# debbiemarkslab/BEAR

Measured on AMD Instinct MI355X. Metric: k-mer contexts/sec (DM-marginal+grad h), k=13, higher is better.
Workload: dtype f64

## Files before the change

bear_amd/csrc/kernels_plan.h:

```cpp
#pragma once
#include "plan_common.h"

__global__ __launch_bounds__(256) void plan_scan_kernel(const uint32_t *__restrict__ counts, uint64_t n_rows, int ncol,
                                                        uint8_t *__restrict__ quad_light,
                                                        unsigned long long *__restrict__ heavy_counts,
                                                        unsigned long long *__restrict__ hist) {
  __shared__ uint32_t s_heavy[3];
  __shared__ uint32_t s_hist[2 * SRT_NKEY];
  __shared__ uint32_t s_big[PLN_NBIG + 1];
  __shared__ unsigned long long s_total, s_cells;
  __shared__ uint32_t s_cmax;
  unsigned long long my_total = 0ull;
  uint32_t my_cells = 0u, my_cmax = 0u;
  if (threadIdx.x == 0) {
    s_total = s_cells = 0ull;
    s_cmax = 0u;
  }
  if (threadIdx.x < 3) s_heavy[threadIdx.x] = 0;
  if (threadIdx.x < 2 * SRT_NKEY) s_hist[threadIdx.x] = 0;
  for (uint32_t k = threadIdx.x; k <= PLN_NBIG; k += 256) s_big[k] = 0;
  __syncthreads();
  const uint64_t n_quads = (n_rows + PLN_QUAD - 1) / PLN_QUAD;
  for (uint64_t g = (uint64_t)blockIdx.x * 256 + threadIdx.x; g < n_quads; g += (uint64_t)gridDim.x * 256) {
    uint32_t light = 0, qhc = 0, qhr = 0;
// ... 156 lines not shown
    meta[2] = run > 0xffffffffull ? 1ull : 0ull;
  }
  __syncthreads();
  unsigned long long off = part[threadIdx.x];
  for (uint64_t t = lo; t < hi; ++t) {
    tiles[t].off16 = (uint32_t)off;
    off += tiles[t].blk16;
  }
}

__global__ __launch_bounds__(1024) void plan_fill_kernel(const uint32_t *__restrict__ counts, uint64_t n_rows, int ncol,
                                                         const pln_tile *__restrict__ tiles, uint64_t n_tiles,
                                                         unsigned char *__restrict__ stream,
                                                         pln_heavy_col *__restrict__ heavy_col,
                                                         pln_heavy_row *__restrict__ heavy_row,
                                                         uint64_t *__restrict__ heavy_stop,
                                                         unsigned long long *__restrict__ cursors) {
  constexpr int RPT = (PLN_RMAX + 1023) / 1024;
  __shared__ uint32_t hist[SRT_NHIST];
  __shared__ uint32_t offs[SRT_NHIST];
  __shared__ uint32_t scan[16];
  __shared__ uint16_t sorted[PLN_NI + 64];
  __shared__ uint32_t s_hc, s_hr;
#ifdef BEAR_DET_BUILD
  __shared__ uint32_t comp[PLN_NI];
  static_assert((PLN_NI & (PLN_NI - 1)) == 0 && PLN_NI <= 2048, "bitonic sort over the tile's items: PLN_NI / 2 pairs, at most one per thread");
  __shared__ unsigned long long hkey[PLN_HCAP], htmp[PLN_HCAP];
#endif
  const uint32_t tid = threadIdx.x, rep = tid & (SRT_REP - 1);
  for (uint64_t t = blockIdx.x; t < n_tiles; t += gridDim.x) {
    const pln_tile ti = tiles[t];
    const uint32_t rows = ti.rows_items >> 16, n_light = ti.rows_items & 0xffffu;
    const uint32_t hc_cap = ti.hc_hr >> 16, hr_cap = ti.hc_hr & 0xffffu;
    const pln_layout L = pln_block_layout(rows, n_light, hc_cap, hr_cap);
    unsigned char *blk = stream + (size_t)ti.off16 * 16;
    uint16_t *E = reinterpret_cast<uint16_t *>(blk);
    uint8_t *nrow = blk + L.nrow;
    uint16_t *items = reinterpret_cast<uint16_t *>(blk + L.items);
    uint16_t *hoff = reinterpret_cast<uint16_t *>(blk + L.hoff);
    uint32_t *hcnt = reinterpret_cast<uint32_t *>(blk + L.hcnt);
    uint16_t *hrow = reinterpret_cast<uint16_t *>(blk + L.hrow);
    double *hn = reinterpret_cast<double *>(blk + L.hn);
    if (tid < SRT_NHIST) hist[tid] = 0;
    if (tid == 0) {
      s_hc = 0;
      s_hr = 0;
    }
    __syncthreads();
#ifdef BEAR_DET_BUILD
    uint32_t det_hc[RPT], det_hr[RPT];
    {
      uint32_t base_c = 0, base_r = 0;
#pragma unroll
      for (int k = 0; k < RPT; ++k) {
        const uint32_t lr = tid + 1024u * k;
        uint32_t nc = 0, nr = 0;
        if (lr < rows) {
          double n = 0.0;
          for (int b = 0; b < 5; ++b) {
            const uint32_t cv = counts[(ti.row0 + lr) * 5 + b];
            n += (double)cv;
            nc += (b < ncol && cv > SRT_CL) ? 1u : 0u;
          }
          nr = n > (double)SRT_CL ? 1u : 0u;
        }
        const uint32_t packed = nc | (nr << 16);
        const int lane = tid & 63, wave = tid >> 6;
        uint32_t incl = packed;
#pragma unroll
        for (int off = 1; off < 64; off <<= 1) {
          const uint32_t o = (uint32_t)__shfl_up((int)incl, off, 64);
          if (lane >= off) incl += o;
        }
        __syncthreads();
        if (lane == 63) scan[wave] = incl;
        __syncthreads();
        uint32_t before = 0, total = 0;
        for (int w = 0; w < 16; ++w) {
          if (w < wave) before += scan[w];
          total += scan[w];
        }
        const uint32_t excl = before + incl - packed;
        det_hc[k] = base_c + (excl & 0xffffu);
        det_hr[k] = base_r + (excl >> 16);
        base_c += total & 0xffffu;
        base_r += total >> 16;
      }
      __syncthreads();
      if (tid == 0) {
        s_hc = base_c;
        s_hr = base_r;
      }
    }
#endif
    uint32_t c[RPT][5], rank[RPT][5];
#pragma unroll
    for (int k = 0; k < RPT; ++k) {
      const uint32_t lr = tid + 1024u * k;
#pragma unroll
      for (int b = 0; b < 5; ++b) {
        c[k][b] = 0;
        rank[k][b] = 0;
      }
      if (lr < rows) {
        const uint64_t r = ti.row0 + lr;
        double n = 0.0;
#pragma unroll
        for (int b = 0; b < 5; ++b) {
          c[k][b] = counts[r * 5 + b];
          n += (double)c[k][b];
        }
        nrow[lr] = n < 1.0 ? (uint8_t)0 : (n <= (double)SRT_CL ? (uint8_t)n : (uint8_t)255);
        if (n > (double)SRT_CL) {
#ifdef BEAR_DET_BUILD
          const uint32_t k2 = hr_cap ? det_hr[k] : 0xffffffffu;
#else
          const uint32_t k2 = hr_cap ? atomicAdd(&s_hr, 1u) : 0xffffffffu;
#endif
          if (k2 < hr_cap) {
            hrow[k2] = (uint16_t)lr;
            hn[k2] = n;
          } else {
            const unsigned long long q = atomicAdd(&cursors[1], 1ull);
            heavy_row[q].row = r;
            heavy_row[q].n = n;
          }
        }
        if (ncol == 4 && c[k][4] > SRT_CL) heavy_stop[atomicAdd(&cursors[2], 1ull)] = c[k][4];
#pragma unroll
        for (int b = 0; b < 5; ++b) {
          if (b >= ncol) c[k][b] = 0;
          if (c[k][b] > SRT_CL) {
#ifdef BEAR_DET_BUILD
            const uint32_t k2 = hc_cap ? det_hc[k]++ : 0xffffffffu;
#else
            const uint32_t k2 = hc_cap ? atomicAdd(&s_hc, 1u) : 0xffffffffu;
#endif
            if (k2 < hc_cap) {
              hoff[k2] = (uint16_t)(lr * 5 + b);
              hcnt[k2] = c[k][b];
            } else {
              const unsigned long long q = atomicAdd(&cursors[0], 1ull);
              heavy_col[q].off = r * 5 + b;
              heavy_col[q].c = c[k][b];
            }
            c[k][b] = 0;
          }
          if (c[k][b] != 0) rank[k][b] = atomicAdd(&hist[(c[k][b] - 1) * SRT_REP + rep], 1u);
        }
      } else if (lr < ((rows + 15u) & ~15u)) {
        nrow[lr] = 0;
      }
    }
    __syncthreads();
    {
      const uint32_t v = tid < SRT_NHIST ? hist[tid] : 0u;
      const int lane = tid & 63, wave = tid >> 6;
      uint32_t incl = v;
#pragma unroll
      for (int off = 1; off < 64; off <<= 1) {
        uint32_t o = (uint32_t)__shfl_up((int)incl, off, 64);
        if (lane >= off) incl += o;
      }
      if (lane == 63) scan[wave] = incl;
      __syncthreads();
      uint32_t base = 0;
      for (int w = 0; w < wave; ++w) base += scan[w];
      if (tid < SRT_NHIST) offs[tid] = base + incl - v;
    }
    __syncthreads();
    if (tid < 30) E[tid] = (uint16_t)(tid < SRT_CL ? offs[tid * SRT_REP] : n_light);
    if (tid == 30) E[30] = (uint16_t)hc_cap;
    if (tid == 31) E[31] = (uint16_t)hr_cap;
#pragma unroll
    for (int k = 0; k < RPT; ++k)
#pragma unroll
      for (int b = 0; b < 5; ++b)
        if (c[k][b] != 0) sorted[offs[(c[k][b] - 1) * SRT_REP + rep] + rank[k][b]] = (uint16_t)((tid + 1024u * k) * 5 + b);
    __syncthreads();
#ifdef BEAR_DET_BUILD
    {
      for (uint32_t i = tid; i < PLN_NI; i += 1024) {
        uint32_t key = 0;
        for (uint32_t q = 1; q < SRT_CL; ++q) key += offs[q * SRT_REP] <= i ? 1u : 0u;
        comp[i] = i < n_light ? (key << 16) | sorted[i] : 0xffffffffu;
      }
      __syncthreads();
      for (uint32_t size = 2; size <= PLN_NI; size <<= 1)
        for (uint32_t stride = size >> 1; stride > 0; stride >>= 1) {
          const uint32_t lo = 2u * tid - (tid & (stride - 1u)), hi = lo + stride;
          if (tid < PLN_NI / 2) {
            const bool up = (lo & size) == 0u;
            const uint32_t a = comp[lo], bq = comp[hi];
            if ((a > bq) == up) {
              comp[lo] = bq;
              comp[hi] = a;
            }
          }
          __syncthreads();
        }
      for (uint32_t i = tid; i < n_light; i += 1024) sorted[i] = (uint16_t)(comp[i] & 0xffffu);
      __syncthreads();
      const uint32_t nhc = s_hc < hc_cap ? s_hc : hc_cap, nhr = s_hr < hr_cap ? s_hr : hr_cap;
      if (tid < nhc) hkey[tid] = ((unsigned long long)hoff[tid] << 32) | hcnt[tid];
      __syncthreads();
      if (tid < nhc) {
        uint32_t r = 0;
        for (uint32_t q = 0; q < nhc; ++q) r += hkey[q] < hkey[tid] ? 1u : 0u;
        htmp[r] = hkey[tid];
      }
      __syncthreads();
      if (tid < nhc) {
        hoff[tid] = (uint16_t)(htmp[tid] >> 32);
        hcnt[tid] = (uint32_t)htmp[tid];
      }
      __syncthreads();
      if (tid < nhr) hkey[tid] = ((unsigned long long)hrow[tid] << 48) | tid;
      if (tid < nhr) htmp[tid] = (unsigned long long)__double_as_longlong(hn[tid]);
      __syncthreads();
      uint32_t r = 0;
      unsigned long long mine = 0ull, myn = 0ull;
      if (tid < nhr) {
        for (uint32_t q = 0; q < nhr; ++q) r += hkey[q] < hkey[tid] ? 1u : 0u;
        mine = hkey[tid];
        myn = htmp[tid];
      }
      __syncthreads();
      if (tid < nhr) {
        hrow[r] = (uint16_t)(mine >> 48);
        hn[r] = __longlong_as_double((long long)myn);
      }
      __syncthreads();
    }
#endif
    const uint32_t padded = (n_light + 63u) & ~63u;
    for (uint32_t i = tid; i < padded; i += 1024) items[i] = i < n_light ? sorted[i] : (uint16_t)PLN_SENTINEL;
    __syncthreads();
  }
}

__global__ __launch_bounds__(1024) void plan_live_kernel(const pln_tile *__restrict__ tiles, uint64_t n_tiles,
                                                         const unsigned char *__restrict__ stream, uint16_t *__restrict__ live) {
  constexpr int RPT = (PLN_RMAX + 1023) / 1024;
  __shared__ uint32_t cnt[RPT * 16];
  const uint32_t tid = threadIdx.x, lane = tid & 63, wave = tid >> 6;
  for (uint64_t t = blockIdx.x; t < n_tiles; t += gridDim.x) {
    const pln_tile ti = tiles[t];
    const uint32_t rows = ti.rows_items >> 16;
    const uint8_t *nrow = stream + (size_t)ti.off16 * 16 + 64;
    uint16_t *out = live + t * PLN_LIVE_STRIDE;
    unsigned long long mask[RPT];
#pragma unroll
    for (int k = 0; k < RPT; ++k) {
      const uint32_t lr = tid + 1024u * k;
      mask[k] = __builtin_amdgcn_ballot_w64(lr < rows && nrow[lr] != 0);
      if (lane == 0) cnt[k * 16 + wave] = (uint32_t)__builtin_popcountll(mask[k]);
    }
    __syncthreads();
    uint32_t total = 0;
#pragma unroll
    for (int k = 0; k < RPT; ++k) {
      uint32_t base = total;
      for (int w = 0; w < 16; ++w) {
        const uint32_t c = cnt[k * 16 + w];
        if (w < (int)wave) base += c;
        total += c;
      }
      if ((mask[k] >> lane) & 1ull) out[1 + base + (uint32_t)__builtin_popcountll(mask[k] & ((1ull << lane) - 1ull))] = (uint16_t)(tid + 1024u * k);
    }
    if (tid == 0) out[0] = (uint16_t)total;
    __syncthreads();
  }
}

template <bool NORM, bool AR>
__global__ __launch_bounds__(PLN_THREADS, 4) void dm_prior_plan_kernel(const double *__restrict__ prior,
                                                                                    uint64_t n_rows, bear_params prm_arg,
                                                                                    pln_view pv,
                                                                                    const double2 *__restrict__ logtab_g,
                                                                                    double *__restrict__ partials,
                                                                                    const bear_step_io io
#ifdef PLN_STAMPS
                                                                                    , unsigned long long *__restrict__ dbg
#endif
                                                                                    ) {
  extern __shared__ __attribute__((aligned(16))) unsigned char srt_smem[];
  pln_lds_n &S = *reinterpret_cast<pln_lds_n *>(srt_smem);
  const bear_params prm = bear_params_of(prm_arg, io);
  const uint32_t tid = threadIdx.x, lane = tid & 63, wave = srt_uniform(tid >> 6);
  const double u = prm.inv_h, eps = prm.eps, eps5 = 5.0 * prm.eps;
  double acc[2] = {0.0, 0.0};

  if (tid < BEAR_LOGTAB_N) S.logtab[tid] = logtab_g[tid];
  if (tid < SRT_NKEY) {
    const bear_dp o = srt_general_fast(u + eps5, (double)(tid + 1), logtab_g);
    S.tabD[tid] = o.D;
    S.tabP[tid] = o.P;
  }
  if (tid < PLN_NBUF) {
    S.buf[tid].pri[PLN_SENTINEL] = 1.0;
    S.ticket[tid] = PLN_TICKET_START(PLN_WAVES - PLN_DMA_WAVES);
    S.sum_fail[tid] = 0xffffffffu;
  }

  const bool dma_wave = wave >= PLN_WAVES - PLN_DMA_WAVES;
  const uint32_t dw = wave - (PLN_WAVES - PLN_DMA_WAVES);
  constexpr bool GEN = !NORM && !AR;
  constexpr bool NT = GEN && PLN_GEN_NT;
  auto stage = [&](const pln_tile &ti, uint32_t b, bool with_nrow) {
    const uint32_t rows = ti.rows_items >> 16;
    if (rows == 0) return;
    const uint32_t pbytes = (rows * 40u) & ~15u, bbytes = ti.blk16 * 16u;
    const unsigned char *psrc = reinterpret_cast<const unsigned char *>(prior + ti.row0 * 5);
    const unsigned char *bsrc = pv.stream + (size_t)ti.off16 * 16;
    if (GEN && dw == 0 && lane == 0) S.nrow_in[b] = with_nrow ? 1u : 0u;
    if (!GEN || with_nrow) {
      for (uint32_t pc = dw; (pc << 10) < bbytes; pc += PLN_DMA_WAVES) pln_dma_piece<NT>(S.buf[b].blk, bsrc, bbytes, pc, lane);
    } else {
      const uint32_t items0 = pln_block_layout(rows, ti.rows_items & 0xffffu, ti.hc_hr >> 16, ti.hc_hr & 0xffffu).items;
      if (dw == PLN_DMA_WAVES - 1) pln_dma_piece<NT>(S.buf[b].blk, bsrc, 64u, 0u, lane);
      for (uint32_t pc = dw; (pc << 10) < bbytes - items0; pc += PLN_DMA_WAVES)
        pln_dma_piece<NT>(S.buf[b].blk + items0, bsrc + items0, bbytes - items0, pc, lane);
    }
    for (uint32_t pc = dw; (pc << 10) < pbytes; pc += PLN_DMA_WAVES) pln_dma_piece<NT>(S.buf[b].pri, psrc, pbytes, pc, lane);
    if (dw == 0 && ((rows * 40u) & 15u)) {
      const __attribute__((address_space(4))) double *tail =
          (const __attribute__((address_space(4))) double *)(uintptr_t)(prior + (ti.row0 + rows) * 5 - 1);
      const double v = *tail;
      if (lane == 0) S.buf[b].pri[rows * 5 - 1] = v;
    }
  };

  constexpr uint32_t PF_INSTR = (NORM || AR || PLN_GEN_PREFETCH) ? PLN_PREFETCH_KIB / 8u : 0u;
  auto prefetch_behind = [&](const pln_tile &ti) -> uint32_t {
    const uint32_t rows = ti.rows_items >> 16;
    if (PF_INSTR == 0 || rows == 0) return 0u;
    const uint64_t end_bytes = n_rows * 40ull, base = (ti.row0 + rows) * 40ull;
    const uint32_t m = srt_uniform((uint32_t)(uintptr_t)S.pf_scratch);
    uint32_t issued = 0;
    for (uint32_t k = dw; k < PF_INSTR; k += PLN_DMA_WAVES) {
      uint64_t off = base + ((uint64_t)(k * 64u + lane) << 7);
      if (off + 4u > end_bytes) off = end_bytes - 4u;
      const unsigned char *g = reinterpret_cast<const unsigned char *>(prior) + off;
      uint32_t keep_m0;
      asm volatile("s_mov_b32 %0, m0\n\ts_mov_b32 m0, %2\n\ts_nop 0\n\tglobal_load_lds_dword %1, off\n\ts_mov_b32 m0, %0"
                   : "=&s"(keep_m0)
                   : "v"(g), "s"(m)
                   : "memory");
      ++issued;
    }
    return issued;
  };
  uint32_t pf_young = 0;
#ifdef PLN_STAMPS
  unsigned long long tph[8] = {0, 0, 0, 0, 0, 0, 0, 0}, t_prev = __builtin_amdgcn_s_memtime();
  int prev_kind = 0;
#define PLN_STAMP(k)                                              \
  {                                                               \
    const unsigned long long now = __builtin_amdgcn_s_memtime();  \
    tph[k] += now - t_prev;                                       \
    t_prev = now;                                                 \
  }
#else
#define PLN_STAMP(k)
#endif
  static_assert(PLN_NBUF == 2, "the DMA-wave protocol below is written for a two-slot ring");
  const uint64_t G = gridDim.x;
  const uint64_t first = (pv.n_tiles * (uint64_t)blockIdx.x) / G, count = (pv.n_tiles * ((uint64_t)blockIdx.x + 1)) / G - first;
  auto fetch_desc = [&](uint64_t j0) {
    if (dw == 0 && j0 < count)
      pln_dma_piece(S.desc[(j0 >> 5) & 1u], pv.tiles + first + j0, PLN_DESC_CHUNK * (uint32_t)sizeof(pln_tile), 0u, lane);
  };
  if (dma_wave) {
    __builtin_amdgcn_s_setprio(3);
    fetch_desc(0);
    fetch_desc(PLN_DESC_CHUNK);
    srt_wait_dma();
  }
  __syncthreads();
  pln_tile cur = pln_desc(S.desc, 0, count), nxt = pln_desc(S.desc, 1, count);
  if (dma_wave) stage(cur, 0, !PLN_GEN_NROW_ON_DEMAND);
  uint32_t slot = 0;
  for (uint64_t j = 0; j < count; ++j) {
#ifdef PLN_STAMPS
    PLN_STAMP(prev_kind)
    prev_kind = 4;
#endif
    if (dma_wave) pln_wait_all_but(pf_young);
    PLN_STAMP(1)
    srt_sync();
    PLN_STAMP(2)
    const pln_tile nn = pln_desc(S.desc, j + 2, count);
    if (dma_wave) {
      if ((j & (PLN_DESC_CHUNK - 1)) == 0 && j != 0) fetch_desc(j + PLN_DESC_CHUNK);
      stage(nxt, slot ^ 1u, !GEN || !PLN_GEN_NROW_ON_DEMAND || srt_uniform(S.sum_fail[slot ^ 1u]) == (uint32_t)j);
      pf_young = prefetch_behind(nxt);
      cur = nxt;
      nxt = nn;
      slot ^= 1u;
      continue;
    }
    PLN_STAMP(3)

    const pln_buf_n &B = S.buf[slot];
    const uint32_t rows = cur.rows_items >> 16, n_light = cur.rows_items & 0xffffu;
    const uint32_t hc = cur.hc_hr >> 16, hr = cur.hc_hr & 0xffffu;
    const pln_layout L = pln_block_layout(rows, n_light, hc, hr);
    const uint16_t *E = reinterpret_cast<const uint16_t *>(B.blk);
    const uint8_t *nrow = B.blk + L.nrow;
    const uint16_t *items = reinterpret_cast<const uint16_t *>(B.blk + L.items);
    if (tid == 0) S.ticket[(slot + 1) % PLN_NBUF] = PLN_TICKET_START(PLN_WAVES - PLN_DMA_WAVES);
    const uint32_t n_hcu = (hc + 63u) >> 6, n_hru = AR ? 0u : (hr + 63u) >> 6, n_heavy = n_hcu + n_hru;
    const uint32_t n_units = (n_light + 63u) >> 6;
    const uint32_t n_work = n_heavy + n_units;
    static_assert(PLN_CHUNK == 128, "two adjacent contexts per lane");
    for (uint32_t c = wave; GEN && c * PLN_CHUNK < rows; c += PLN_WAVES - PLN_DMA_WAVES) {
      const uint32_t row0c = c * PLN_CHUNK + 2u * lane;
      const uint32_t rr = row0c < rows ? row0c : 0u;
      const double2 *src = reinterpret_cast<const double2 *>(&B.pri[rr * 5]);
      const double2 v0 = src[0], v1 = src[1], v2 = src[2], v3 = src[3], v4 = src[4];
      const double S5[2] = {((v0.x + v0.y) + (v1.x + v1.y)) + v2.x, ((v2.y + v3.x) + (v3.y + v4.x)) + v4.y};
      bool bad[2];
#pragma unroll
      for (int q = 0; q < 2; ++q) bad[q] = row0c + q < rows && !(__builtin_fabs(S5[q] - 1.0) <= SRT_SUM1_TOL);
      if (__builtin_amdgcn_ballot_w64(bad[0] || bad[1])) {
        if (lane == 0) S.sum_fail[slot] = (uint32_t)(j + 1);
        uint32_t nn_[2];
        if (!PLN_GEN_NROW_ON_DEMAND || srt_uniform(S.nrow_in[slot])) {
#pragma unroll
          for (int q = 0; q < 2; ++q) nn_[q] = bad[q] ? (uint32_t)nrow[rr + q] : 0u;
        } else {
          const uint8_t *g = pv.stream + (size_t)cur.off16 * 16 + L.nrow;
#pragma unroll
          for (int q = 0; q < 2; ++q) nn_[q] = bad[q] ? (uint32_t)g[rr + q] : 0u;
        }
#pragma unroll
        for (int q = 0; q < PLN_CHUNK / 64; ++q) {
          const uint32_t own = nn_[q] == 255u ? 0u : nn_[q];
          if (__builtin_amdgcn_ballot_w64(own != 0)) {
            uint32_t cm = own;
#pragma unroll
            for (int off = 32; off > 0; off >>= 1) {
              const uint32_t o2 = (uint32_t)__shfl_xor((int)cm, off, 64);
              cm = o2 > cm ? o2 : cm;
            }
            const double xa[1] = {own ? __builtin_fma(S5[q], u, eps5) : 1.0};
            const uint32_t ca[1] = {own};
            bear_dp o[1];
            srt_light<1>(xa, ca, 0u, srt_uniform(cm), S.logtab, o);
            if (own) {
              acc[0] += S.tabD[own - 1] - o[0].D;
              acc[1] = __builtin_fma(xa[0] - eps5, o[0].P, __builtin_fma(-u, S.tabP[own - 1], acc[1]));
            }
          }
        }
      }
    }
    PLN_FOR_UNITS_F(w, &S.ticket[slot], n_work, wave, PLN_WAVES - PLN_DMA_WAVES) {
#ifdef PLN_STAMPS
      {
        const unsigned long long now = __builtin_amdgcn_s_memtime();
        tph[prev_kind] += now - t_prev;
        t_prev = now;
        prev_kind = w < n_heavy ? 5 : 6;
      }
#endif
      if (w < n_hcu) {
        const uint32_t i = w * 64u + lane;
        if (i < hc) {
          const uint32_t off = reinterpret_cast<const uint16_t *>(B.blk + L.hoff)[i];
          const double cnt = (double)reinterpret_cast<const uint32_t *>(B.blk + L.hcnt)[i];
          if (AR) {
            acc[0] = __builtin_fma(cnt, bear_log_tab(B.pri[off] + eps, S.logtab), acc[0]);
          } else {
            const double x = __builtin_fma(B.pri[off], u, eps);
            const bear_dp o = srt_general_fast(x, cnt, S.logtab);
            acc[0] += o.D;
            acc[1] = __builtin_fma(eps - x, o.P, acc[1]);
          }
        }
        continue;
      }
      if (w < n_heavy) {
        const uint32_t i = (w - n_hcu) * 64u + lane;
        if (i < hr) {
          const double *f = &B.pri[(uint32_t)reinterpret_cast<const uint16_t *>(B.blk + L.hrow)[i] * 5u];
          const double A = NORM ? u + eps5 : __builtin_fma(((f[0] + f[1]) + (f[2] + f[3])) + f[4], u, eps5);
          const bear_dp o = srt_general_fast(A, reinterpret_cast<const double *>(B.blk + L.hn)[i], S.logtab);
          acc[0] -= o.D;
          acc[1] = __builtin_fma(A - eps5, o.P, acc[1]);
        }
        continue;
      }
      {
        const uint32_t un = n_heavy + n_units - 1u - w;
        uint32_t cmin, cmax;
        const uint32_t ci[1] = {pln_unit_counts(E, n_light, un, lane, &cmin, &cmax)};
        const uint32_t off = items[un * 64u + lane];
        if (AR) {
          acc[0] = __builtin_fma((double)ci[0], bear_log_tab(B.pri[off] + eps, S.logtab), acc[0]);
          continue;
        }
        const double x[1] = {__builtin_fma(B.pri[off], u, eps)};
        bear_dp o[1];
        srt_light<1>(x, ci, cmin, cmax, S.logtab, o);
        acc[0] += o[0].D;
        acc[1] = __builtin_fma(eps - x[0], o[0].P, acc[1]);
        continue;
      }
    }
    cur = nxt;
    nxt = nn;
    slot ^= 1u;
  }
  srt_wait_dma();
#ifdef PLN_STAMPS
  if (lane == 0 && dbg) {
    for (int k = 0; k < 8; ++k) dbg[((size_t)blockIdx.x * PLN_WAVES + wave) * 8 + k] = tph[k];
  }
#endif
  const uint64_t gtid = (uint64_t)blockIdx.x * PLN_THREADS + tid, gsz = (uint64_t)gridDim.x * PLN_THREADS;
  for (uint64_t i = gtid; i < pv.n_heavy_col; i += gsz) {
    const pln_heavy_col h = pv.heavy_col[i];
    if (AR) {
      acc[0] = __builtin_fma((double)h.c, bear_log_tab(prior[h.off] + eps, S.logtab), acc[0]);
      continue;
    }
    const double x = __builtin_fma(prior[h.off], u, eps);
    const bear_dp o = srt_general_fast(x, (double)h.c, S.logtab);
    acc[0] += o.D;
    acc[1] = __builtin_fma(eps - x, o.P, acc[1]);
  }
  for (uint64_t i = gtid; !AR && i < pv.n_heavy_row; i += gsz) {
    const pln_heavy_row h = pv.heavy_row[i];
    const double *f = prior + h.row * 5;
    const double A = __builtin_fma(((f[0] + f[1]) + (f[2] + f[3])) + f[4], u, eps5);
    const bear_dp o = srt_general_fast(A, h.n, S.logtab);
    acc[0] -= o.D;
    acc[1] = __builtin_fma(A - eps5, o.P, acc[1]);
  }
  if (!AR && blockIdx.x == 0 && tid < SRT_CL) {
    const double m = (double)pv.hist[tid];
    acc[0] -= m * S.tabD[tid];
    acc[1] = __builtin_fma(u * m, S.tabP[tid], acc[1]);
  }
  __syncthreads();
  block_finish<2>(acc, partials, io);
}

struct pln_buf_r {
  uint32_t ref[PLN_RMAX * 5 + 4];
  __attribute__((aligned(16))) unsigned char blk[PLN_BLOCK_MAX];
};
#define PLN_RSLOT 3
struct pln_lds_r {
  pln_buf_r buf[PLN_RSLOT];
  double2 logtab[BEAR_LOGTAB_N];
  double tabD[2][SRT_NKEY];
  double tabP[2][SRT_NKEY];
  uint32_t meta[PLN_RSLOT][2];
  uint32_t ticket[PLN_RSLOT];
  uint32_t landed[PLN_RSLOT];
  uint32_t left[PLN_RSLOT];
};

template <bool AR>
__global__ __launch_bounds__(PLN_THREADS, 4) void dm_ref_plan_kernel(const uint32_t *__restrict__ ref,
                                                                                  uint64_t n_rows, bear_params prm_arg,
                                                                                  pln_view pv,
                                                                                  const double2 *__restrict__ logtab_g,
                                                                                  double *__restrict__ partials,
                                                                                  const bear_step_io io, const bear_apply_io apply) {
  extern __shared__ __attribute__((aligned(16))) unsigned char srt_smem[];
  pln_lds_r &S = *reinterpret_cast<pln_lds_r *>(srt_smem);
  const bear_params prm = bear_params_of(prm_arg, io);
  const uint32_t tid = threadIdx.x, lane = tid & 63, wave = srt_uniform(tid >> 6);
  const double u = prm.inv_h, eps = prm.eps;
  const double A = u + 5.0 * eps;
  const double x4 = prm.nw * prm.V * u + eps;
  const double VU = prm.V * u;
  const double tau = prm.tau;
  const double w2c = tau * (eps + 0.25 * VU);
  const double nwV = prm.nw * prm.V;
  double acc[4] = {0.0, 0.0, 0.0, 0.0};

  if (tid < BEAR_LOGTAB_N) S.logtab[tid] = logtab_g[tid];
  if (tid < 2 * SRT_NKEY) {
    const int which = tid / SRT_NKEY, j = tid % SRT_NKEY;
    const bear_dp o = srt_general_fast(which ? x4 : A, (double)(j + 1), logtab_g);
    S.tabD[which][j] = o.D;
    S.tabP[which][j] = o.P;
  }
  if (tid < PLN_RSLOT) {
    S.landed[tid] = S.left[tid] = 0u;
    S.ticket[tid] = PLN_TICKET_START(PLN_WAVES - PLN_DMA_WAVES);
  }
  if (tid < 4 * PLN_RSLOT) S.buf[tid >> 2].ref[PLN_SENTINEL + (tid & 3)] = 0;

  const bool dma_wave = wave >= PLN_WAVES - PLN_DMA_WAVES;
  const uint32_t dw = wave - (PLN_WAVES - PLN_DMA_WAVES);
  constexpr uint32_t CWAVES = PLN_WAVES - PLN_DMA_WAVES;
  auto stage = [&](const pln_tile &ti, uint32_t b) {
    const uint32_t rows = ti.rows_items >> 16;
    const uint32_t rbytes = rows * 20u, rb16 = rbytes & ~15u, bbytes = ti.blk16 * 16u;
    const unsigned char *rsrc = reinterpret_cast<const unsigned char *>(ref + ti.row0 * 5);
    const unsigned char *bsrc = pv.stream + (size_t)ti.off16 * 16;
    for (uint32_t pc = 0; (pc << 10) < bbytes; ++pc) pln_dma_piece(S.buf[b].blk, bsrc, bbytes, pc, lane);
    for (uint32_t pc = 0; (pc << 10) < rb16; ++pc) pln_dma_piece(S.buf[b].ref, rsrc, rb16, pc, lane);
    if (rbytes & 15u) {
      const uint32_t w0 = rb16 >> 2, nw = (rbytes & 15u) >> 2;
      const __attribute__((address_space(4))) uint32_t *tail =
          (const __attribute__((address_space(4))) uint32_t *)(uintptr_t)(ref + ti.row0 * 5 + w0);
      const uint32_t v0 = tail[0], v1 = nw > 1 ? tail[1] : 0u, v2 = nw > 2 ? tail[2] : 0u;
      if (lane == 0) {
        S.buf[b].ref[w0] = v0;
        if (nw > 1) S.buf[b].ref[w0 + 1] = v1;
        if (nw > 2) S.buf[b].ref[w0 + 2] = v2;
      }
    }
    if (lane == 0) {
      S.meta[b][0] = ti.rows_items;
      S.meta[b][1] = ti.hc_hr;
      S.ticket[b] = PLN_TICKET_START(PLN_WAVES - PLN_DMA_WAVES);
    }
  };
  auto alpha_from = [&](double rb, double R) {
    const double dev = __builtin_fma(rb + eps, bear_rcp(R), -0.25);
    return __builtin_fma(__builtin_fma(prm.E, dev, 0.25), VU, eps);
  };
  auto accumulate = [&](double x, const bear_dp &o) {
    const double w1 = eps - x;
    acc[0] += o.D;
    acc[1] = __builtin_fma(w1, o.P, acc[1]);
    acc[2] = __builtin_fma(__builtin_fma(-tau, x, w2c), o.P, acc[2]);
    acc[3] = __builtin_fma(nwV * w1, o.P, acc[3]);
  };
  auto accumulate_ar = [&](double rb, double R, double c) {
    const double dev = __builtin_fma(rb + eps, bear_rcp(R), -0.25);
    const double f = __builtin_fma(prm.E, dev, 0.25) * prm.V;
    const double p = f + eps;
    const double dLdf = c * bear_rcp(p);
    acc[0] = __builtin_fma(c, bear_log_tab(p, S.logtab), acc[0]);
    acc[2] = __builtin_fma(dLdf, -prm.tauE * dev * prm.V, acc[2]);
    acc[3] = __builtin_fma(dLdf, -nwV * f, acc[3]);
  };

  const uint64_t G = gridDim.x;
  const uint64_t first = (pv.n_tiles * (uint64_t)blockIdx.x) / G, count = (pv.n_tiles * ((uint64_t)blockIdx.x + 1)) / G - first;
  __syncthreads();
  if (dma_wave) {
    __builtin_amdgcn_s_setprio(3);
    pln_tile ti = pln_load_tile(pv, dw < count ? first + dw : pv.n_tiles);
    for (uint64_t j = dw; j < count; j += PLN_DMA_WAVES) {
      const uint32_t b = (uint32_t)(j % PLN_RSLOT), gen = (uint32_t)(j / PLN_RSLOT);
      const pln_tile ti_next = pln_load_tile(pv, j + PLN_DMA_WAVES < count ? first + j + PLN_DMA_WAVES : pv.n_tiles);
      while (pln_peek(&S.left[b]) < CWAVES * gen) __builtin_amdgcn_s_sleep(1);
      stage(ti, b);
      srt_wait_dma();
      asm volatile("s_waitcnt lgkmcnt(0)" ::: "memory");
      if (lane == 0) atomicAdd(&S.landed[b], 1u);
      ti = ti_next;
    }
  }
  for (uint64_t j = 0; !dma_wave && j < count; ++j) {
    const uint32_t slot = (uint32_t)(j % PLN_RSLOT), gen = (uint32_t)(j / PLN_RSLOT);
    while (pln_peek(&S.landed[slot]) < gen + 1u) __builtin_amdgcn_s_sleep(1);
    const pln_buf_r &B = S.buf[slot];
    const uint32_t rows_items = srt_uniform(S.meta[slot][0]), hc_hr = srt_uniform(S.meta[slot][1]);
    const uint32_t rows = rows_items >> 16, n_light = rows_items & 0xffffu;
    const uint32_t hc = hc_hr >> 16;
    const pln_layout L = pln_block_layout(rows, n_light, hc, hc_hr & 0xffffu);
    const uint16_t *E = reinterpret_cast<const uint16_t *>(B.blk);
    const uint16_t *items = reinterpret_cast<const uint16_t *>(B.blk + L.items);
    const uint32_t n_hcu = (hc + 63u) >> 6;
    const uint32_t n_units = (n_light + 63u) >> 6;
    PLN_FOR_UNITS_F(w, &S.ticket[slot], n_hcu + n_units, wave, CWAVES) {
      if (w < n_hcu) {
        const uint32_t i = w * 64u + lane;
        if (i < hc) {
          const uint32_t off = reinterpret_cast<const uint16_t *>(B.blk + L.hoff)[i];
          const uint32_t *rr = &B.ref[((off * 52429u) >> 18) * 5u];
          const double R = (double)(((uint64_t)rr[0] + rr[1]) + ((uint64_t)rr[2] + rr[3])) + 4.0 * eps;
          const double cnt = (double)reinterpret_cast<const uint32_t *>(B.blk + L.hcnt)[i];
          if (AR) {
            accumulate_ar((double)B.ref[off], R, cnt);
          } else {
            const double x = alpha_from((double)B.ref[off], R);
            accumulate(x, srt_general_fast(x, cnt, S.logtab));
          }
        }
        continue;
      }
      const uint32_t un = n_hcu + n_units - 1u - w;
      uint32_t cmin, cmax;
      const uint32_t ci[1] = {pln_unit_counts(E, n_light, un, lane, &cmin, &cmax)};
      const uint32_t off = items[un * 64u + lane];
      const uint32_t *rr = &B.ref[((off * 52429u) >> 18) * 5u];
      const double R = (double)(((uint64_t)rr[0] + rr[1]) + ((uint64_t)rr[2] + rr[3])) + 4.0 * eps;
      if (AR) {
        accumulate_ar((double)B.ref[off], R, (double)ci[0]);
        continue;
      }
      const double x[1] = {alpha_from((double)B.ref[off], R)};
      bear_dp o[1];
      srt_light<1>(x, ci, cmin, cmax, S.logtab, o);
      accumulate(x[0], o[0]);
    }
    asm volatile("s_waitcnt lgkmcnt(0)" ::: "memory");
    if (lane == 0) atomicAdd(&S.left[slot], 1u);
  }
  srt_wait_dma();
  const uint64_t gtid = (uint64_t)blockIdx.x * PLN_THREADS + tid, gsz = (uint64_t)gridDim.x * PLN_THREADS;
  for (uint64_t i = gtid; i < pv.n_heavy_col; i += gsz) {
    const pln_heavy_col h = pv.heavy_col[i];
    const uint32_t *rr = ref + (h.off / 5) * 5;
    const double R = (double)(((uint64_t)rr[0] + rr[1]) + ((uint64_t)rr[2] + rr[3])) + 4.0 * eps;
    if (AR) {
      accumulate_ar((double)ref[h.off], R, (double)h.c);
      continue;
    }
    const double x = alpha_from((double)ref[h.off], R);
    accumulate(x, srt_general_fast(x, (double)h.c, S.logtab));
  }
  if (AR) {
    const double f4 = nwV, p4 = f4 + eps;
    double c4sum = 0.0;
    if (blockIdx.x == 0 && tid < SRT_CL) c4sum = (double)(tid + 1) * (double)pv.hist[SRT_NKEY + tid];
    for (uint64_t i = gtid; i < pv.n_heavy_stop; i += gsz) c4sum += (double)pv.heavy_stop[i];
    acc[0] = __builtin_fma(c4sum, bear_log_tab(p4, S.logtab), acc[0]);
    acc[3] = __builtin_fma(c4sum * bear_rcp(p4), nwV * (1.0 - f4), acc[3]);
    __syncthreads();
    block_finish<4>(acc, partials, io, apply);
    return;
  }
  for (uint64_t i = gtid; i < pv.n_heavy_row; i += gsz) {
    const double n = pv.heavy_row[i].n;
    if (pln_in_big_hist(pv, n)) continue;
    const bear_dp o = srt_general_fast(A, n, S.logtab);
    acc[0] -= o.D;
    acc[1] = __builtin_fma(u, o.P, acc[1]);
  }
  pln_big_totals(pv, A, u, gtid, gsz, S.logtab, acc[0], acc[1]);
  for (uint64_t i = gtid; i < pv.n_heavy_stop; i += gsz) {
    const bear_dp o = srt_general_fast(x4, (double)pv.heavy_stop[i], S.logtab);
    acc[0] += o.D;
    acc[1] = __builtin_fma(eps - x4, o.P, acc[1]);
    acc[3] = __builtin_fma(VU * nwV, o.P, acc[3]);
  }
  if (blockIdx.x == 0 && tid < SRT_CL) {
    const double mn = (double)pv.hist[tid], m4 = (double)pv.hist[SRT_NKEY + tid];
    acc[0] -= mn * S.tabD[0][tid];
    acc[1] = __builtin_fma(u * mn, S.tabP[0][tid], acc[1]);
    const double P4 = m4 * S.tabP[1][tid];
    acc[0] += m4 * S.tabD[1][tid];
    acc[1] = __builtin_fma(eps - x4, P4, acc[1]);
    acc[3] = __builtin_fma(VU * nwV, P4, acc[3]);
  }
  __syncthreads();
  block_finish<4>(acc, partials, io, apply);
}

struct pln_lds_g {
  double pri[PLN_RMAX * 5 + 2];
  double grad[PLN_RMAX * 5 + 2];
  __attribute__((aligned(16))) unsigned char blk[PLN_BLOCK_MAX];
  double2 logtab[BEAR_LOGTAB_N];
  double tabD[SRT_NKEY];
  double tabP[SRT_NKEY];
  uint32_t ticket;
  __attribute__((aligned(16))) uint32_t pf_scratch[64];
};
static_assert(sizeof(pln_lds_g) <= 158 * 1024, "gradient-row kernel: LDS budget");

__device__ __forceinline__ void pln_touch_lines(uint32_t *scratch, const void *src, uint32_t bytes, uint32_t k, uint32_t lane) {
  const uint32_t off = (k * 64u + lane) << 7;
  if (off < bytes) {
    const unsigned char *g = static_cast<const unsigned char *>(src) + off;
    const uint32_t m = srt_uniform((uint32_t)(uintptr_t)scratch);
    uint32_t keep_m0;
    asm volatile("s_mov_b32 %0, m0\n\ts_mov_b32 m0, %2\n\ts_nop 0\n\tglobal_load_lds_dword %1, off\n\ts_mov_b32 m0, %0"
                 : "=&s"(keep_m0)
                 : "v"(g), "s"(m)
                 : "memory");
  }
}

template <bool NORM, bool AR>
__global__ __launch_bounds__(PLN_THREADS, 4) void dm_prior_plan_grad_kernel(const double *__restrict__ prior,
                                                                                         bear_params prm_arg, pln_view pv,
                                                                                         const double2 *__restrict__ logtab_g,
                                                                                         double *__restrict__ grad_out,
                                                                                         double *__restrict__ partials,
                                                                                         const bear_step_io io) {
  extern __shared__ __attribute__((aligned(16))) unsigned char srt_smem[];
  pln_lds_g &S = *reinterpret_cast<pln_lds_g *>(srt_smem);
  const bear_params prm = bear_params_of(prm_arg, io);
  const uint32_t tid = threadIdx.x, lane = tid & 63, wave = srt_uniform(tid >> 6);
  const double u = prm.inv_h, eps = prm.eps, eps5 = 5.0 * prm.eps;
  double acc[2] = {0.0, 0.0};
  if (tid < BEAR_LOGTAB_N) S.logtab[tid] = logtab_g[tid];
  if (tid < SRT_NKEY) {
    const bear_dp o = srt_general_fast(u + eps5, (double)(tid + 1), logtab_g);
    S.tabD[tid] = o.D;
    S.tabP[tid] = o.P;
  }
  if (tid == 0) {
    S.pri[PLN_SENTINEL] = 1.0;
    S.ticket = PLN_TICKET_START(PLN_WAVES);
  }
  pln_tile nxt = pln_load_tile(pv, blockIdx.x);
  for (uint64_t t = blockIdx.x; t < pv.n_tiles; t += gridDim.x) {
    const pln_tile cur = nxt;
    const uint32_t rows = cur.rows_items >> 16, n_light = cur.rows_items & 0xffffu;
// ... 315 lines not shown
```

bear_amd/csrc/plan_common.h:

```cpp
#pragma once
#include "sorted_common.h"

#ifndef PLN_THREADS
#define PLN_THREADS 1024
#endif
#define PLN_WAVES (PLN_THREADS / 64)
#ifndef PLN_UNITS
#define PLN_UNITS 32
#endif
#define PLN_NI (PLN_UNITS * 64)
#ifndef PLN_NI_CUT
#define PLN_NI_CUT PLN_NI
#endif
#ifndef PLN_RMAX
#define PLN_RMAX 1664
#endif
#ifndef PLN_HCAP
#define PLN_HCAP 128
#endif
#define PLN_NBIG 4096
#define PLN_BLOCKS_PER_CU (1024 / PLN_THREADS)
#define PLN_QUAD 4
#define PLN_LIVE_STRIDE (PLN_RMAX + 8)
#define PLN_SENTINEL (PLN_RMAX * 5)
#ifndef PLN_NBUF
#define PLN_NBUF 2
#endif
#define PLN_BLOCK_MAX (64 + PLN_RMAX + PLN_NI * 2 + PLN_HCAP * (2 + 4 + 2 + 8))

struct pln_tile {
  uint64_t row0;
  uint32_t rows_items;
  uint32_t off16;
  uint32_t hc_hr;
  uint32_t blk16;
  uint64_t pad;
};
static_assert(sizeof(pln_tile) == 32, "tile descriptors are fetched with one s_load_dwordx8");
#ifndef PLN_CHUNK
#define PLN_CHUNK 128
#endif
#ifndef PLN_DMA_WAVES
#define PLN_DMA_WAVES 2
#endif
#ifndef PLN_PREFETCH_KIB
#define PLN_PREFETCH_KIB 24
#endif
#ifndef PLN_GEN_PREFETCH
#define PLN_GEN_PREFETCH 1
#endif
#ifndef PLN_GEN_NT
#define PLN_GEN_NT 0
#endif
#ifndef PLN_GEN_NROW_ON_DEMAND
#define PLN_GEN_NROW_ON_DEMAND 1
#endif
#define PLN_DESC_CHUNK 32
#define PLN_DESC_PAD (2 * PLN_DESC_CHUNK)

struct pln_layout {
  uint32_t nrow, items, hoff, hcnt, hrow, hn, end;
};
__host__ __device__ inline pln_layout pln_block_layout(uint32_t rows, uint32_t n_light, uint32_t hc, uint32_t hr) {
  pln_layout L;
  L.nrow = 64u;
  L.items = L.nrow + ((rows + 15u) & ~15u);
  L.hoff = L.items + (((n_light + 63u) & ~63u) * 2u);
  L.hcnt = L.hoff + (((hc + 7u) & ~7u) * 2u);
  L.hrow = L.hcnt + (((hc + 3u) & ~3u) * 4u);
  L.hn = L.hrow + (((hr + 7u) & ~7u) * 2u);
  L.end = L.hn + (((hr + 1u) & ~1u) * 8u);
  return L;
}

struct pln_heavy_col {
  uint64_t off;
  uint64_t c;
};

struct pln_heavy_row {
  uint64_t row;
  double n;
};

struct pln_view {
  const pln_tile *tiles;
  const unsigned char *stream;
  const pln_heavy_col *heavy_col;
  const pln_heavy_row *heavy_row;
  const uint64_t *heavy_stop;
  const unsigned long long *hist;
  const unsigned long long *hist_big;
  int big_in_hist;
  uint64_t n_tiles, n_heavy_col, n_heavy_row, n_heavy_stop;
  const uint16_t *live;
  const uint16_t *live2;
  int subset;
};

__device__ __forceinline__ void pln_big_totals(const pln_view &pv, double A, double scale, uint64_t gtid, uint64_t gsz, const double2 *logtab,
                                               double &acc_D, double &acc_P) {
  if (!pv.hist_big) return;
  for (uint64_t n = SRT_CL + 1 + gtid; n <= PLN_NBIG; n += gsz) {
    const unsigned long long m = pv.hist_big[n];
    if (m) {
      const bear_dp o = srt_general_fast(A, (double)n, logtab);
      acc_D -= (double)m * o.D;
      acc_P = __builtin_fma(scale * (double)m, o.P, acc_P);
    }
  }
}
__device__ __forceinline__ bool pln_in_big_hist(const pln_view &pv, double n) { return pv.big_in_hist && n <= (double)PLN_NBIG; }

__device__ __forceinline__ uint32_t pln_dma(void *lds, const void *src, uint32_t bytes, uint32_t wave, uint32_t lane,
                                            uint32_t first) {
  const uint32_t d = (uint32_t)(uintptr_t)lds;
  const unsigned char *s = static_cast<const unsigned char *>(src) + lane * 16u;
  const uint32_t pieces = (bytes + 1023u) >> 10;
  uint32_t issued = 0;
  for (uint32_t piece = (wave + PLN_WAVES - (first % PLN_WAVES)) % PLN_WAVES; piece < pieces; piece += PLN_WAVES) {
    const unsigned char *g = s + (piece << 10);
    const uint32_t m = srt_uniform(d + (piece << 10));
    if ((piece << 10) + lane * 16u < bytes)
      {
      uint32_t keep_m0;
      asm volatile("s_mov_b32 %0, m0\n\ts_mov_b32 m0, %2\n\ts_nop 0\n\tglobal_load_lds_dwordx4 %1, off\n\ts_mov_b32 m0, %0"
                   : "=&s"(keep_m0)
                   : "v"(g), "s"(m)
                   : "memory");
    }
    ++issued;
  }
  return issued;
}

template <bool NT = false>
__device__ __forceinline__ void pln_dma_piece(void *lds, const void *src, uint32_t bytes, uint32_t piece, uint32_t lane) {
  const uint32_t m = srt_uniform((uint32_t)(uintptr_t)lds + (piece << 10));
  const unsigned char *g = static_cast<const unsigned char *>(src) + (piece << 10) + lane * 16u;
  if ((piece << 10) + lane * 16u < bytes)
    {
      uint32_t keep_m0;
      if (NT)
        asm volatile("s_mov_b32 %0, m0\n\ts_mov_b32 m0, %2\n\ts_nop 0\n\tglobal_load_lds_dwordx4 %1, off nt\n\ts_mov_b32 m0, %0"
                     : "=&s"(keep_m0)
                     : "v"(g), "s"(m)
                     : "memory");
      else
        asm volatile("s_mov_b32 %0, m0\n\ts_mov_b32 m0, %2\n\ts_nop 0\n\tglobal_load_lds_dwordx4 %1, off\n\ts_mov_b32 m0, %0"
                     : "=&s"(keep_m0)
                     : "v"(g), "s"(m)
                     : "memory");
    }
}

__device__ __forceinline__ void pln_wait_all_but(uint32_t younger) {
  switch (younger) {
    case 0: asm volatile("s_waitcnt vmcnt(0)" ::: "memory"); break;
    case 1: asm volatile("s_waitcnt vmcnt(1)" ::: "memory"); break;
    case 2: asm volatile("s_waitcnt vmcnt(2)" ::: "memory"); break;
    case 3: asm volatile("s_waitcnt vmcnt(3)" ::: "memory"); break;
    case 4: asm volatile("s_waitcnt vmcnt(4)" ::: "memory"); break;
    case 5: asm volatile("s_waitcnt vmcnt(5)" ::: "memory"); break;
    case 6: asm volatile("s_waitcnt vmcnt(6)" ::: "memory"); break;
    case 7: asm volatile("s_waitcnt vmcnt(7)" ::: "memory"); break;
    case 8: asm volatile("s_waitcnt vmcnt(8)" ::: "memory"); break;
    default: asm volatile("s_waitcnt vmcnt(0)" ::: "memory"); break;
  }
}

__device__ __forceinline__ pln_tile pln_load_tile(const pln_view &pv, uint64_t t) {
  pln_tile ti;
  ti.row0 = 0;
  ti.rows_items = 0;
  ti.off16 = 0;
  ti.hc_hr = 0;
  ti.blk16 = 0;
  ti.pad = 0;
  if (t < pv.n_tiles) {
    const __attribute__((address_space(4))) pln_tile *tc = (const __attribute__((address_space(4))) pln_tile *)(uintptr_t)pv.tiles;
    ti.row0 = tc[t].row0;
    ti.rows_items = tc[t].rows_items;
    ti.off16 = tc[t].off16;
    ti.hc_hr = tc[t].hc_hr;
    ti.blk16 = tc[t].blk16;
    ti.pad = tc[t].pad;
  }
  return ti;
}

__device__ __forceinline__ uint32_t pln_ticket(uint32_t *counter, uint32_t lane) {
  uint32_t t = 0;
  if (lane == 0)
    asm volatile("ds_add_rtn_u32 %0, %1, %2\n\ts_waitcnt lgkmcnt(0)" : "=&v"(t) : "v"((uint32_t)(uintptr_t)counter), "v"(1u) : "memory");
  return srt_uniform(t);
}

#ifdef BEAR_DET_BUILD
#define PLN_FOR_UNITS(w, counter, n, first, stride) for (uint32_t w = (first); w < (n); w += (stride))
#else
#define PLN_FOR_UNITS(w, counter, n, first, stride) for (uint32_t w = pln_ticket(counter, lane); w < (n); w = pln_ticket(counter, lane))
#endif
#if defined(BEAR_DET_BUILD) || defined(PLN_NO_FIRST_UNIT_DEALT)
#define PLN_FOR_UNITS_F(w, counter, n, first, stride) PLN_FOR_UNITS(w, counter, n, first, stride)
#define PLN_TICKET_START(stride) 0u
#else
#define PLN_FOR_UNITS_F(w, counter, n, first, stride) for (uint32_t w = (first); w < (n); w = pln_ticket(counter, lane))
#define PLN_TICKET_START(stride) ((uint32_t)(stride))
#endif

__device__ __forceinline__ uint32_t pln_ticket_issue(uint32_t *counter, uint32_t lane) {
  uint32_t t = 0;
  if (lane == 0) t = atomicAdd(counter, 1u);
  return t;
}

__device__ __forceinline__ uint32_t pln_unit_counts(const uint16_t *E, uint32_t n_light, uint32_t un, uint32_t lane,
                                                    uint32_t *cmin, uint32_t *cmax) {
  const uint32_t base = un * 64u, idx = base + lane;
  const uint32_t last = (base + 64u <= n_light ? base + 64u : n_light) - 1u;
  const uint32_t e = lane < 30u ? (uint32_t)E[lane] : 0xffffffffu;
  uint32_t lo, hi;
  asm("s_bcnt1_i32_b64 %0, %1" : "=s"(lo) : "s"(__builtin_amdgcn_ballot_w64(e <= base)) : "scc");
  asm("s_bcnt1_i32_b64 %0, %1" : "=s"(hi) : "s"(__builtin_amdgcn_ballot_w64(e <= last)) : "scc");
  uint32_t c = lo;
  for (uint32_t k = lo; k < hi; ++k) c += idx >= (uint32_t)__builtin_amdgcn_readlane((int)e, (int)k) ? 1u : 0u;
  *cmin = base + 64u <= n_light ? lo : 0u;
  *cmax = hi;
  return idx < n_light ? c : 0u;
}

struct pln_buf_n {
  double pri[PLN_RMAX * 5 + 2];
  __attribute__((aligned(16))) unsigned char blk[PLN_BLOCK_MAX];
};
struct pln_lds_n {
  pln_buf_n buf[PLN_NBUF];
  double2 logtab[BEAR_LOGTAB_N];
  double tabD[SRT_NKEY];
  double tabP[SRT_NKEY];
  uint32_t ticket[PLN_NBUF];
  uint32_t sum_fail[PLN_NBUF];
  uint32_t nrow_in[PLN_NBUF];
  __attribute__((aligned(16))) pln_tile desc[2][PLN_DESC_CHUNK];
  __attribute__((aligned(16))) uint32_t pf_scratch[64];
};
static_assert(sizeof(pln_lds_n) <= 160 * 1024, "one block per CU: the planned mode-N kernels' LDS");

__device__ __forceinline__ pln_tile pln_desc(const pln_tile (*ring)[PLN_DESC_CHUNK], uint64_t j, uint64_t count) {
  pln_tile ti;
  ti.row0 = 0;
  ti.rows_items = 0;
  ti.off16 = 0;
  ti.hc_hr = 0;
  ti.blk16 = 0;
  ti.pad = 0;
  if (j < count) {
    const uint32_t *d = reinterpret_cast<const uint32_t *>(&ring[(j >> 5) & 1u][j & 31u]);
    const uint32_t lo = srt_uniform(d[0]), hi = srt_uniform(d[1]);
    ti.row0 = ((uint64_t)hi << 32) | lo;
    ti.rows_items = srt_uniform(d[2]);
    ti.off16 = srt_uniform(d[3]);
    ti.hc_hr = srt_uniform(d[4]);
    ti.blk16 = srt_uniform(d[5]);
  }
  return ti;
}

__device__ __forceinline__ uint32_t pln_peek(const uint32_t *p) {
  return srt_uniform(__hip_atomic_load(p, __ATOMIC_RELAXED, __HIP_MEMORY_SCOPE_WORKGROUP));
}
```

Measured before the change: 134.1 billion.

## Bucket sum-failing rows by count into sorted work units for balanced light evaluation

When the previous tile on a buffer had rows whose prior sums deviate from one, each compute wave now builds a per-count histogram of those rows, scans it, and scatters row indices into a sorted list. That list is then processed as extra ticketed work units through the existing light-path evaluator, replacing the per-chunk loop that shuffled for the max count and ran divergent srt_light calls. This adds LDS state, atomics, spin-wait arrival counters and a more complex work loop, in exchange for better lane utilization on tiles with many unnormalized rows.

```diff
diff --git a/bear_amd/csrc/kernels_plan.h b/bear_amd/csrc/kernels_plan.h
--- a/bear_amd/csrc/kernels_plan.h
+++ b/bear_amd/csrc/kernels_plan.h
@@ -482,11 +482,21 @@
     S.ticket[tid] = PLN_TICKET_START(PLN_WAVES - PLN_DMA_WAVES);
     S.sum_fail[tid] = 0xffffffffu;
   }
+  if (!NORM && !AR && tid < PLN_NBUF) S.own_arrived[tid] = 0u;
+  if (!NORM && !AR && tid < PLN_NBUF * (SRT_CL + 1)) (&S.own_hist[0][0])[tid] = 0u;
 
   const bool dma_wave = wave >= PLN_WAVES - PLN_DMA_WAVES;
   const uint32_t dw = wave - (PLN_WAVES - PLN_DMA_WAVES);
   constexpr bool GEN = !NORM && !AR;
   constexpr bool NT = GEN && PLN_GEN_NT;
+  constexpr uint32_t CWAVES = PLN_WAVES - PLN_DMA_WAVES;
+#ifdef BEAR_DET_BUILD
+  constexpr bool SORTED = false;
+#else
+  constexpr bool SORTED = GEN && PLN_GEN_NROW_ON_DEMAND && CWAVES * PLN_CHUNK >= PLN_RMAX;
+#endif
+  bool prev_sorted = false;
+  bool sorted_next = false;
   auto stage = [&](const pln_tile &ti, uint32_t b, bool with_nrow) {
     const uint32_t rows = ti.rows_items >> 16;
     if (rows == 0) return;
@@ -570,6 +580,7 @@
     PLN_STAMP(1)
     srt_sync();
     PLN_STAMP(2)
+    const uint32_t fail_v = SORTED ? S.sum_fail[slot ^ 1u] : 0u;
     const pln_tile nn = pln_desc(S.desc, j + 2, count);
     if (dma_wave) {
       if ((j & (PLN_DESC_CHUNK - 1)) == 0 && j != 0) fetch_desc(j + PLN_DESC_CHUNK);
@@ -592,9 +603,53 @@
     if (tid == 0) S.ticket[(slot + 1) % PLN_NBUF] = PLN_TICKET_START(PLN_WAVES - PLN_DMA_WAVES);
     const uint32_t n_hcu = (hc + 63u) >> 6, n_hru = AR ? 0u : (hr + 63u) >> 6, n_heavy = n_hcu + n_hru;
     const uint32_t n_units = (n_light + 63u) >> 6;
-    const uint32_t n_work = n_heavy + n_units;
+    uint32_t n_work = n_heavy + n_units;
+    const bool own_sorted = SORTED && sorted_next;
+    if (SORTED && prev_sorted) {
+      if (tid <= SRT_CL) S.own_hist[slot ^ 1u][tid] = 0u;
+      if (tid == 0) S.own_arrived[slot ^ 1u] = 0u;
+    }
+    uint32_t own_total = 0, own[2] = {0u, 0u}, rank[2] = {0u, 0u};
+    if (SORTED && own_sorted) {
+      if (wave * PLN_CHUNK < rows) {
+        const uint32_t row0c = wave * PLN_CHUNK + 2u * lane;
+        const uint32_t rr = row0c < rows ? row0c : 0u;
+        const double2 *src = reinterpret_cast<const double2 *>(&B.pri[rr * 5]);
+        const double2 v0 = src[0], v1 = src[1], v2 = src[2], v3 = src[3], v4 = src[4];
+        const uint32_t n2 = *reinterpret_cast<const uint16_t *>(nrow + rr);
+        const double S5[2] = {((v0.x + v0.y) + (v1.x + v1.y)) + v2.x, ((v2.y + v3.x) + (v3.y + v4.x)) + v4.y};
+        bool bad[2];
+#pragma unroll
+        for (int q = 0; q < 2; ++q) bad[q] = row0c + q < rows && !(__builtin_fabs(S5[q] - 1.0) <= SRT_SUM1_TOL);
+        if (__builtin_amdgcn_ballot_w64(bad[0] || bad[1])) {
+          if (lane == 0) S.sum_fail[slot] = (uint32_t)(j + 1);
+#pragma unroll
+          for (int q = 0; q < 2; ++q) {
+            const uint32_t n = bad[q] ? (n2 >> (8 * q)) & 0xffu : 0u;
+            own[q] = n > SRT_CL ? 0u : n;
+            if (own[q]) rank[q] = atomicAdd(&S.own_hist[slot][own[q]], 1u);
+          }
+        }
+      }
+      pln_arrive(&S.own_arrived[slot], lane);
+    }
+    auto own_scatter = [&]() {
+      while (pln_peek(&S.own_arrived[slot]) < CWAVES) __builtin_amdgcn_s_sleep(1);
+      asm volatile("" ::: "memory");
+      const uint32_t incl = pln_scan_lo32(lane >= 1u && lane <= SRT_CL ? S.own_hist[slot][lane] : 0u, lane);
+      own_total = (uint32_t)__builtin_amdgcn_readlane((int)incl, 31);
+      if (wave == 0 && lane < 32u) S.own_E[lane] = (uint16_t)incl;
+      const uint32_t row0c = wave * PLN_CHUNK + 2u * lane;
+#pragma unroll
+      for (int q = 0; q < 2; ++q) {
+        const uint32_t at = (uint32_t)__shfl((int)incl, own[q] ? (int)own[q] - 1 : 0, 64) + rank[q];
+        if (own[q]) S.own_list[at < PLN_RMAX ? at : PLN_RMAX - 1u] = (uint16_t)(row0c + q);
+      }
+      pln_arrive(&S.own_arrived[slot], lane);
+      n_work += (own_total + 63u) >> 6;
+    };
     static_assert(PLN_CHUNK == 128, "two adjacent contexts per lane");
-    for (uint32_t c = wave; GEN && c * PLN_CHUNK < rows; c += PLN_WAVES - PLN_DMA_WAVES) {
+    for (uint32_t c = wave; GEN && !own_sorted && c * PLN_CHUNK < rows; c += PLN_WAVES - PLN_DMA_WAVES) {
       const uint32_t row0c = c * PLN_CHUNK + 2u * lane;
       const uint32_t rr = row0c < rows ? row0c : 0u;
       const double2 *src = reinterpret_cast<const double2 *>(&B.pri[rr * 5]);
@@ -636,7 +691,7 @@
         }
       }
     }
-    PLN_FOR_UNITS_F(w, &S.ticket[slot], n_work, wave, PLN_WAVES - PLN_DMA_WAVES) {
+    auto unit = [&](uint32_t w) {
 #ifdef PLN_STAMPS
       {
         const unsigned long long now = __builtin_amdgcn_s_memtime();
@@ -659,7 +714,7 @@
             acc[1] = __builtin_fma(eps - x, o.P, acc[1]);
           }
         }
-        continue;
+        return;
       }
       if (w < n_heavy) {
         const uint32_t i = (w - n_hcu) * 64u + lane;
@@ -670,7 +725,25 @@
           acc[0] -= o.D;
           acc[1] = __builtin_fma(A - eps5, o.P, acc[1]);
         }
-        continue;
+        return;
+      }
+      if (SORTED && w >= n_heavy + n_units) {
+        while (pln_peek(&S.own_arrived[slot]) < 2u * CWAVES) __builtin_amdgcn_s_sleep(1);
+        asm volatile("" ::: "memory");
+        const uint32_t un = n_work - 1u - w;
+        uint32_t cmin, cmax;
+        const uint32_t ci[1] = {pln_unit_counts(S.own_E, own_total, un, lane, &cmin, &cmax)};
+        const uint32_t row = S.own_list[un * 64u + lane];
+        const double *f = &B.pri[(ci[0] ? row : 0u) * 5u];
+        const double s5 = ((f[0] + f[1]) + (f[2] + f[3])) + f[4];
+        const double x[1] = {ci[0] ? __builtin_fma(s5, u, eps5) : 1.0};
+        bear_dp o[1];
+        srt_light<1>(x, ci, cmin, cmax, S.logtab, o);
+        if (ci[0]) {
+          acc[0] += S.tabD[ci[0] - 1] - o[0].D;
+          acc[1] = __builtin_fma(x[0] - eps5, o[0].P, __builtin_fma(-u, S.tabP[ci[0] - 1], acc[1]));
+        }
+        return;
       }
       {
         const uint32_t un = n_heavy + n_units - 1u - w;
@@ -679,16 +752,35 @@
         const uint32_t off = items[un * 64u + lane];
         if (AR) {
           acc[0] = __builtin_fma((double)ci[0], bear_log_tab(B.pri[off] + eps, S.logtab), acc[0]);
-          continue;
+          return;
         }
         const double x[1] = {__builtin_fma(B.pri[off], u, eps)};
         bear_dp o[1];
         srt_light<1>(x, ci, cmin, cmax, S.logtab, o);
         acc[0] += o[0].D;
         acc[1] = __builtin_fma(eps - x[0], o[0].P, acc[1]);
-        continue;
-      }
-    }
+        return;
+      }
+    };
+    if (!(SORTED && own_sorted)) {
+      PLN_FOR_UNITS_F(w, &S.ticket[slot], n_work, wave, CWAVES) unit(w);
+    } else {
+      uint32_t w = wave;
+      for (bool due = true;;) {
+        const bool run = w < n_work;
+        if (run) unit(w);
+        if (due) {
+          own_scatter();
+          due = false;
+          if (!run) continue;
+        } else if (!run) {
+          break;
+        }
+        w = pln_ticket(&S.ticket[slot], lane);
+      }
+    }
+    prev_sorted = own_sorted;
+    sorted_next = SORTED && srt_uniform(fail_v) == (uint32_t)j;
     cur = nxt;
     nxt = nn;
     slot ^= 1u;
diff --git a/bear_amd/csrc/plan_common.h b/bear_amd/csrc/plan_common.h
--- a/bear_amd/csrc/plan_common.h
+++ b/bear_amd/csrc/plan_common.h
@@ -244,6 +244,10 @@
   uint32_t nrow_in[PLN_NBUF];
   __attribute__((aligned(16))) pln_tile desc[2][PLN_DESC_CHUNK];
   __attribute__((aligned(16))) uint32_t pf_scratch[64];
+  uint32_t own_hist[PLN_NBUF][SRT_CL + 1];
+  uint32_t own_arrived[PLN_NBUF];
+  uint16_t own_E[32];
+  uint16_t own_list[PLN_RMAX + 64];
 };
 static_assert(sizeof(pln_lds_n) <= 160 * 1024, "one block per CU: the planned mode-N kernels' LDS");
 
@@ -267,6 +271,19 @@
   return ti;
 }
 
+__device__ __forceinline__ void pln_arrive(uint32_t *counter, uint32_t lane) {
+  if (lane == 0) asm volatile("ds_add_u32 %0, %1" : : "v"((uint32_t)(uintptr_t)counter), "v"(1u) : "memory");
+}
+
+__device__ __forceinline__ uint32_t pln_scan_lo32(uint32_t v, uint32_t lane) {
+  v += (uint32_t)__builtin_amdgcn_update_dpp(0, (int)v, 0x111, 0xf, 0xf, true);
+  v += (uint32_t)__builtin_amdgcn_update_dpp(0, (int)v, 0x112, 0xf, 0xf, true);
+  v += (uint32_t)__builtin_amdgcn_update_dpp(0, (int)v, 0x114, 0xf, 0xf, true);
+  v += (uint32_t)__builtin_amdgcn_update_dpp(0, (int)v, 0x118, 0xf, 0xf, true);
+  const uint32_t row0 = (uint32_t)__builtin_amdgcn_readlane((int)v, 15);
+  return lane >= 16u ? v + row0 : v;
+}
+
 __device__ __forceinline__ uint32_t pln_peek(const uint32_t *p) {
   return srt_uniform(__hip_atomic_load(p, __ATOMIC_RELAXED, __HIP_MEMORY_SCOPE_WORKGROUP));
 }
```

Result: no change. 134.5 billion, median of 6 (+0.3%).
